# AwesomePeiweiPan/Droid-SLAM_Reserch

Hardware: AMD Instinct MI355X
Metric: BA update iters/sec (2000-edge equivalents; 256 keyframes, 48x64) (higher is better)
Workload: dtype f32; 1 GPU; 256-keyframe / 2000-edge global BA, 48x64, t0=1, lm=1e-5 ep=1e-2 (BASELINE configs[2]); edges_total=2000, solve=fp64 dense Cholesky on device, chol_failed=False

## Files before the change

### droid-slam_reserch_amd/csrc/ba_internal.hpp

```cpp
#pragma once
#include <hip/hip_runtime.h>
#include <stddef.h>
#include <stdint.h>

namespace droid {

constexpr int LIN_THREADS = 256;
constexpr int LIN_PPT = 2;
constexpr int LIN_CP = LIN_THREADS * LIN_PPT;
constexpr int LIN_WAVES = LIN_THREADS / 64;
constexpr int CHOL_NB = 64;
__host__ __device__ inline int chol_ld(int n) { return (n + 1 + 15) & ~15; }
__host__ __device__ inline size_t chol_flag_words(int n) { return 2 * ((size_t)(n + 1 + CHOL_NB - 1) / CHOL_NB) + 8; }
__host__ __device__ inline int chol_tile_index(int nrb, int bi, int bj) { return bj * nrb - bj * (bj - 1) / 2 + (bi - bj); }
__host__ __device__ inline size_t chol_tiles(int n) {
  const int nb = (n + CHOL_NB - 1) / CHOL_NB, nrb = (n + 1 + CHOL_NB - 1) / CHOL_NB;
  return (size_t)chol_tile_index(nrb, nb, nb);
}
__host__ __device__ inline size_t chol_mbuf_offset(int n) { return ((size_t)(n + CHOL_NB - 1) / CHOL_NB) * CHOL_NB * CHOL_NB; }
__host__ __device__ inline size_t chol_lfin_offset(int n) { return 2 * chol_mbuf_offset(n); }
__host__ __device__ inline size_t chol_ldiag_doubles(int n) { return chol_lfin_offset(n) + chol_tiles(n) * CHOL_NB * CHOL_NB; }

__host__ __device__ inline size_t pk_colbase(int n, int J) {
  return (size_t)CHOL_NB * ((size_t)J * (size_t)(n + 1) - (size_t)CHOL_NB * (size_t)J * (size_t)(J - 1) / 2);
}
__host__ __device__ inline int pk_width(int n, int J) { return (n - CHOL_NB * J) < CHOL_NB ? (n - CHOL_NB * J) : CHOL_NB; }
__host__ __device__ inline size_t pk_total(int n) {
  if (n <= 0) return 0;
  const int nb = (n + CHOL_NB - 1) / CHOL_NB;
  return pk_colbase(n, nb - 1) + (size_t)(n + 1 - CHOL_NB * (nb - 1)) * (size_t)pk_width(n, nb - 1);
}
__host__ __device__ inline size_t pk_index(int n, int gi, int gj) {
  const int J = gj / CHOL_NB;
  return pk_colbase(n, J) + (size_t)(gi - CHOL_NB * J) * (size_t)pk_width(n, J) + (size_t)(gj - CHOL_NB * J);
}
__host__ __device__ inline unsigned pk_index32(int n, int gi, int gj) {
  const int J = gj >> 6, c0 = J << 6;
  const int w = (n - c0) < CHOL_NB ? (n - c0) : CHOL_NB;
  return (unsigned)(CHOL_NB * (J * (n + 1) - (CHOL_NB / 2) * J * (J - 1)) + (gi - c0) * w + (gj - c0));
}

enum { HDR_STATUS = 0, HDR_M = 1, HDR_CHOL_FAIL = 2, HDR_NENT = 3, HDR_NWORK = 4,
       HDR_NC1 = 5, HDR_NC2 = 6,
       HDR_WORDS = 16 };
enum { STATUS_BAD_INDEX = 1, STATUS_ETA_ROWS = 2, STATUS_CHOL_FAIL = 4, STATUS_CHOL_STALL = 8 };

struct BaView {
  int E, nbuf, H, W, HW;
  int t0, t1, P, M;
  int n, ld;
  int nch;
  int own0, own1;
  int motion_only;
  int* hdr;
  int* slot_of;
  int* kx;
  int* seg_ptr;
  int* seg_edge;
  int* cursor;
  int* ent_ptr;
  int* ent_row;
  int* ent_pose;
  int* wk_ptr;
  int* order;
  int* xtmp;
  int* cls_list;
  int* gt_ptr;
  double* Gpart;
  int s2_split;
  float* Hpart;
  float* Q;
  float* w;
  float* Erows;
  float* Ebuf;
  float* sy_part[2];
  int sy_ns[2];
  int wide;
  int zsplit;
  float* zpart;
  double* sys;
  double* psys;
  int packed;
  double* xsol;
  float* dx;
  int* bs_flags;
  double* ldiag;
  int* hint;
  int hint_tag;
  int* ov_ready;
};

constexpr int SY_WGS = 1024;
constexpr int S2_WGS = 1536;
constexpr int SF_WGS = 1536;
constexpr int LIN_WGS = 1536;
constexpr int LIN_ZERO_WGS = 192;
constexpr int SF_TP = 64;
constexpr int SW_MID = 256;
constexpr int SW_BIG = 512;
constexpr int tri_tiles16(int rows) { return (rows / 16) * (rows / 16 + 1) / 2; }
constexpr int SY_T1 = tri_tiles16(SW_MID), SY_T2 = tri_tiles16(SW_BIG);
constexpr int SY_FOLD_GROUPS = SY_T1 / 4;

inline size_t ba_carve(BaView& v, void* ws, int E, int nbuf, int H, int W, int t0, int t1, int M) {
  v.E = E; v.nbuf = nbuf; v.H = H; v.W = W; v.HW = H * W;
  v.t0 = t0; v.t1 = t1; v.P = t1 - t0; v.M = M;
  v.n = 6 * v.P; v.ld = chol_ld(v.n);
  v.nch = (v.HW + LIN_CP - 1) / LIN_CP;
  v.own0 = 0; v.own1 = nbuf; v.motion_only = 0;
  v.hint = nullptr; v.hint_tag = 0;
  size_t off = 0;
  char* base = static_cast<char*>(ws);
  auto take = [&](size_t bytes) {
    void* p = base ? base + off : nullptr;
    off += (bytes + 255) & ~size_t(255);
    return p;
  };
  v.hdr = static_cast<int*>(take(sizeof(int) * HDR_WORDS));
  v.slot_of = static_cast<int*>(take(sizeof(int) * (nbuf + 1)));
  v.kx = static_cast<int*>(take(sizeof(int) * (nbuf + 1)));
  v.seg_ptr = static_cast<int*>(take(sizeof(int) * (nbuf + 2)));
  v.seg_edge = static_cast<int*>(take(sizeof(int) * (E + 1)));
  v.cursor = static_cast<int*>(take(sizeof(int) * (nbuf + 2)));
  v.ent_ptr = static_cast<int*>(take(sizeof(int) * (nbuf + 2)));
  v.ent_row = static_cast<int*>(take(sizeof(int) * ((size_t)M + E + 1)));
  v.ent_pose = static_cast<int*>(take(sizeof(int) * ((size_t)M + E + 1)));
  v.wk_ptr = static_cast<int*>(take(sizeof(int) * (nbuf + 2)));
  v.order = static_cast<int*>(take(sizeof(int) * (nbuf + 2)));
  v.gt_ptr = static_cast<int*>(take(sizeof(int) * (nbuf + 2)));
  v.cls_list = static_cast<int*>(take(sizeof(int) * 2 * (nbuf + 2)));
  v.xtmp = static_cast<int*>(take(sizeof(int) * 3 * ((size_t)E + 1)));
  v.Hpart = static_cast<float*>(take(sizeof(float) * ((size_t)E * v.nch * LIN_WAVES * 32 + 32)));
  v.Q = static_cast<float*>(take(sizeof(float) * ((size_t)M * v.HW + 4)));
  v.w = static_cast<float*>(take(sizeof(float) * ((size_t)M * v.HW + 4)));
  v.Erows = nullptr;
  v.wide = (M > 0 && (long)E >= 12l * M && (v.HW % 32) == 0) ? 1 : 0;
  v.Ebuf = nullptr;
  if (v.wide) v.Ebuf = static_cast<float*>(take(sizeof(float) * (6 * ((size_t)M + E) * v.HW + 64)));
  v.sy_part[0] = v.sy_part[1] = nullptr;
  v.sy_ns[0] = v.sy_ns[1] = 0;
  if (v.wide) {
    const int stages = v.HW / 32;
    int nsw = (SY_WGS + M - 1) / M, nsb = (256 + 4 * M - 1) / (4 * M);
    nsw = nsw < 2 ? 2 : (nsw > stages ? stages : nsw);
    nsb = nsb < 2 ? 2 : (nsb > stages ? stages : nsb);
    if (nsw > 16) nsw = 16;
    if (nsb > 16) nsb = 16;
    v.sy_ns[0] = nsw; v.sy_ns[1] = nsb;
    v.sy_part[0] = static_cast<float*>(take(sizeof(float) * ((size_t)M * nsw * SY_T1 * 256 + 64)));
    v.sy_part[1] = static_cast<float*>(take(sizeof(float) * ((size_t)M * nsb * SY_T2 * 256 + 64)));
  }
  v.zsplit = 1;
  if (M > 0) {
    const int z = LIN_WGS / (M * v.nch);
    v.zsplit = z < 1 ? 1 : (z > 8 ? 8 : z);
  }
  v.zpart = nullptr;
  if (v.zsplit > 1) v.zpart = static_cast<float*>(take(sizeof(float) * ((size_t)v.zsplit * M * 8 * v.HW + 64)));
  v.s2_split = 1;
  v.Gpart = nullptr;
  if (M > 0) {
    const int ptiles = (v.HW + 63) / 64;
    int ns = S2_WGS / M;
    v.s2_split = ns < 1 ? 1 : (ns > ptiles ? ptiles : ns);
    size_t tiles = (size_t)E * 7 / 4 + (size_t)M + 1;
    if (tiles > (size_t)28 * M) tiles = (size_t)28 * M;
    v.Gpart = static_cast<double*>(take(sizeof(double) * (tiles * v.s2_split * 256 + 64)));
  }
  v.sys = static_cast<double*>(take(sizeof(double) * ((size_t)(v.n + 1) * v.ld + 8)));
  v.psys = static_cast<double*>(take(sizeof(double) * (pk_total(v.n) + 8)));
  v.packed = 0;
  v.xsol = static_cast<double*>(take(sizeof(double) * ((size_t)v.ld + 1)));
  v.bs_flags = static_cast<int*>(take(sizeof(int) * chol_flag_words(v.n)));
  v.ldiag = static_cast<double*>(take(sizeof(double) * chol_ldiag_doubles(v.n)));
  v.dx = static_cast<float*>(take(sizeof(float) * ((size_t)v.n + 8)));
  v.ov_ready = static_cast<int*>(take(sizeof(int) * ((size_t)(v.n + 1 + CHOL_NB - 1) / CHOL_NB + 8)));
  return off;
}

__host__ __device__ inline int solver_preset_words(const BaView& v) {
  return (int)((reinterpret_cast<const char*>(v.bs_flags) - reinterpret_cast<const char*>(v.xsol)) / 4 +
               (long)chol_flag_words(v.n));
}
__host__ __device__ inline int solver_preset_tiles(const BaView& v) { return v.n > 0 ? (int)chol_tiles(v.n) : 0; }

struct BaLaunchPlan {
  int zero_wgs;
  int asm_units;
  dim3 schur2;
  int sf_split;
  dim3 syrk[2], fold;
};
inline BaLaunchPlan ba_launch_plan(const BaView& v) {
  BaLaunchPlan p;
  p.zero_wgs = LIN_ZERO_WGS;
  p.asm_units = v.E > 0 ? v.E + (solver_preset_words(v) + 1023) / 1024 + solver_preset_tiles(v) : 0;
  p.schur2 = dim3(v.M + (p.asm_units + 4 * v.s2_split - 1) / (4 * v.s2_split), v.s2_split);
  const int tiles = (v.HW + SF_TP - 1) / SF_TP, ns = SF_WGS / (v.M > 0 ? v.M : 1);
  p.sf_split = ns < 1 ? 1 : (ns > tiles ? tiles : ns);
  p.syrk[0] = dim3(v.M, v.sy_ns[0], 1);
  p.syrk[1] = dim3(v.M, v.sy_ns[1], 4);
  p.fold = dim3(v.M, SY_FOLD_GROUPS, 2);
  return p;
}

struct CholSystem {
  double* S; int n, ld; double* x; int* flags; double* ldiag; int* fail;
  explicit CholSystem(const BaView& v)
      : S(v.sys), n(v.n), ld(v.ld), x(v.xsol), flags(v.bs_flags), ldiag(v.ldiag), fail(v.hdr + HDR_CHOL_FAIL) {}
  CholSystem(double* scratch, int n, double* x, int* fail);
  static size_t scratch_doubles(int n);
};

void launch_wave_reduce32_test(const float* in, float* out, hipStream_t s);
void launch_prep(const BaView& v, const int64_t* ii, const int64_t* jj, hipStream_t s);
void launch_unpack_system(const BaView& v, hipStream_t s);
void launch_build_stage(const BaView& v, const BaLaunchPlan& plan, const float* poses, const float* disps,
                        const float* intr, const float* sens, const float* targets, const float* weights,
                        const float* eta, const int64_t* ii, const int64_t* jj, bool motion_only,
                        int stage, hipStream_t s);
void launch_update(const BaView& v, float* poses, float* disps, const float* intr, const float* weights,
                   const int64_t* ii, const int64_t* jj, const double* x, float* dx_out, float* dz_out,
                   bool motion_only, hipStream_t s, int* status_mirror = nullptr);
void launch_chol_preset(const CholSystem& c, hipStream_t s);
bool launch_chol_factor(const CholSystem& c, double lm, double ep, hipStream_t s);
void launch_chol_backsolve(const CholSystem& c, bool factor_single, hipStream_t s);
void launch_chol_solve(const CholSystem& c, double lm, double ep, hipStream_t s, bool preset_done);

void launch_unpack_cols(const BaView& v, int J0, int J1, double lm, double ep, int epoch, hipStream_t s);
bool launch_chol_factor_overlap(const CholSystem& c, const int* ready, int epoch, hipStream_t s);
bool chol_overlap_available(int n);

}
```

### droid-slam_reserch_amd/csrc/ba_kernels.hip

```cpp
#include <hip/hip_runtime.h>
#include <stdint.h>
#include <stdlib.h>

#include "ba_internal.hpp"
#include "se3.hpp"

namespace droid {


__device__ void block_exscan(int* data, int L, int* lds, int* total) {
  const int T = blockDim.x, t = threadIdx.x, lane = t & 63, wave = t >> 6, nw = T >> 6;
  const int per = (L + T - 1) / T;
  const int b = t * per;
  int s = 0;
  for (int k = 0; k < per; k++)
    if (b + k < L) s += data[b + k];
  int incl = s;
#pragma unroll
  for (int off = 1; off < 64; off <<= 1) {
    const int v = __shfl_up(incl, off);
    if (lane >= off) incl += v;
  }
  if (lane == 63) lds[wave] = incl;
  __syncthreads();
  if (wave == 0) {
    int w = (lane < nw) ? lds[lane] : 0;
    int wi = w;
#pragma unroll
    for (int off = 1; off < 64; off <<= 1) {
      const int v = __shfl_up(wi, off);
      if (lane >= off) wi += v;
    }
    if (lane < nw) lds[lane] = wi - w;
    if (lane == nw - 1) *total = wi;
  }
  __syncthreads();
  int run = lds[wave] + incl - s;
  for (int k = 0; k < per; k++)
    if (b + k < L) {
      int v = data[b + k];
      data[b + k] = run;
      run += v;
    }
  __syncthreads();
}

template <int CTRL, int BANKS>
__device__ __forceinline__ float dpp_move(float old, float src) {
  return __int_as_float(__builtin_amdgcn_update_dpp(__float_as_int(old), __float_as_int(src), CTRL, 0xf, BANKS, false));
}
__device__ __forceinline__ float wave_reduce32(float (&v)[32]) {
  constexpr int ROW_SHL4 = 0x104, ROW_SHR4 = 0x114, ROW_ROR8 = 0x128, QUAD_XOR2 = 0x4E, QUAD_XOR1 = 0xB1;
  const int lane = threadIdx.x & 63;
#pragma unroll
  for (int i = 0; i < 16; i++) {
    const auto r = __builtin_amdgcn_permlane32_swap(__float_as_uint(v[2 * i]), __float_as_uint(v[2 * i + 1]), false, false);
    v[i] = __uint_as_float(r[0]) + __uint_as_float(r[1]);
  }
#pragma unroll
  for (int i = 0; i < 8; i++) {
    const auto r = __builtin_amdgcn_permlane16_swap(__float_as_uint(v[2 * i]), __float_as_uint(v[2 * i + 1]), false, false);
    v[i] = __uint_as_float(r[0]) + __uint_as_float(r[1]);
  }
#pragma unroll
  for (int i = 0; i < 4; i++) {
    const float a = dpp_move<ROW_ROR8, 0x3>(v[2 * i + 1], v[2 * i]);
    const float b = dpp_move<ROW_ROR8, 0xC>(v[2 * i], v[2 * i + 1]);
    v[i] = a + b;
  }
#pragma unroll
  for (int i = 0; i < 2; i++) {
    const float a = dpp_move<ROW_SHL4, 0x5>(v[2 * i + 1], v[2 * i]);
    const float b = dpp_move<ROW_SHR4, 0xA>(v[2 * i], v[2 * i + 1]);
    v[i] = a + b;
  }
  {
    const bool hi = lane & 2;
    float keep = hi ? v[1] : v[0];
    float send = hi ? v[0] : v[1];
    v[0] = keep + dpp_move<QUAD_XOR2, 0xF>(send, send);
  }
  return v[0] + dpp_move<QUAD_XOR1, 0xF>(v[0], v[0]);
}

__device__ __forceinline__ int reduce32_index(int lane) {
  return ((lane >> 5) & 1) | (((lane >> 4) & 1) << 1) | (((lane >> 3) & 1) << 2) |
         (((lane >> 2) & 1) << 3) | (((lane >> 1) & 1) << 4);
}

__global__ __launch_bounds__(64) void wave_reduce32_test_kernel(const float* __restrict__ in, float* __restrict__ out) {
  float v[32];
#pragma unroll
  for (int k = 0; k < 32; k++) v[k] = in[threadIdx.x * 32 + k];
  out[threadIdx.x] = wave_reduce32(v);
}
void launch_wave_reduce32_test(const float* in, float* out, hipStream_t s) {
  hipLaunchKernelGGL(wave_reduce32_test_kernel, dim3(1), dim3(64), 0, s, in, out);
}

__device__ __forceinline__ double* sys_at(const BaView& v, int gi, int gj) {
  if (v.packed) {
    unsigned idx = pk_index32(v.n, gi, gj);
    asm volatile("" : "+v"(idx));
    return v.psys + idx;
  }
  return v.sys + (size_t)gi * v.ld + gj;
}

constexpr int SLOT_MAXE = 128;
template <typename S>
struct SlotMetaT {
  int e[SLOT_MAXE];
  int pj[SLOT_MAXE];
  int ent[SLOT_MAXE];
  int flag[SLOT_MAXE];
  S T[SLOT_MAXE][12];
};
typedef SlotMetaT<float> SlotMeta;

constexpr int SF_RB = 96;
constexpr int SY_MAXSPLIT = 16;

constexpr int S2_MAXE = 16;
__device__ __forceinline__ int schur_class(int rows, int nedges, int wide) {
  if (nedges <= S2_MAXE) return 0;
  if (!wide || nedges > SLOT_MAXE || rows > SW_BIG) return 3;
  return rows <= SW_MID ? 1 : 2;
}
__device__ __forceinline__ size_t ebuf_index(int e0, int rows, int HW, int row, int k) {
  return (size_t)6 * e0 * HW + ((size_t)(k >> 5) * rows + row) * 32 + (k & 31);
}
__device__ __forceinline__ int s2_tiles(int nedges) {
  const int ntr = (6 * nedges + 15) / 16;
  return ntr * (ntr + 1) / 2 + 1;
}

template <typename S>
__device__ __forceinline__ void load_slot_meta(SlotMetaT<S>& sm, const BaView& v, const float* __restrict__ poses,
                                               const int64_t* __restrict__ jj, int f, int x0, int cnt,
                                               int ent_base) {
  const int t = threadIdx.x;
  if (t < cnt) {
    const int e = v.seg_edge[x0 + t];
    const int jx = (int)jj[e];
    const RelMat<S> T = rel_pose_mat<S, true>(poses, f, jx);
    sm.e[t] = e;
    sm.pj[t] = jx - v.t0;
    sm.flag[t] = (jx == f) ? 1 : 0;
#pragma unroll
    for (int n = 0; n < 9; n++) sm.T[t][n] = T.R[n];
#pragma unroll
    for (int n = 0; n < 3; n++) sm.T[t][9 + n] = T.t[n];
  }
  __syncthreads();
  if (t < cnt) {
    int a = ent_base;
    for (int u = 0; u < t; u++) a += (sm.pj[u] >= 0 && sm.pj[u] < v.P) ? 1 : 0;
    sm.ent[t] = (sm.pj[t] >= 0 && sm.pj[t] < v.P) ? a : -1;
  }
  __syncthreads();
}

__host__ __device__ inline size_t prep_lds_ints(int nbuf, int E) { return 9 * ((size_t)nbuf + 2) + 4 * ((size_t)E + 1); }

template <bool INLDS>
__global__ __launch_bounds__(1024) void ba_prep_kernel(BaView vg, const int64_t* __restrict__ ii,
                                                        const int64_t* __restrict__ jj) {
  __shared__ int lds[1024];
  __shared__ int tot;
  extern __shared__ int dyn[];
  const int t = threadIdx.x, T = blockDim.x;
  BaView v = vg;
  if (INLDS) {
    int* q = dyn;
    const int nb2 = vg.nbuf + 2, e1 = vg.E + 1;
    v.slot_of = q; q += nb2;
    v.kx = q; q += nb2;
    v.seg_ptr = q; q += nb2;
    v.cursor = q; q += nb2;
    v.ent_ptr = q; q += nb2;
    v.wk_ptr = q; q += nb2;
    v.order = q; q += nb2;
    v.gt_ptr = q; q += nb2;
    q += nb2;
    v.seg_edge = q; q += e1;
    v.xtmp = q;
  }
  const int E = v.E, nbuf = v.nbuf;
  const int w0 = max(v.t0, v.own0), w1 = min(v.t1, v.own1);

  if (t == 0) {
    v.hdr[HDR_STATUS] = 0;
    v.hdr[HDR_CHOL_FAIL] = 0;
  }
  for (int f = t; f < nbuf; f += T) v.slot_of[f] = 0;
  __syncthreads();
  for (int e = t; e < E; e += T) {
    const int64_t i = ii[e], j = jj[e];
    if (i < 0 || i >= nbuf || j < 0 || j >= nbuf)
      atomicOr(&v.hdr[HDR_STATUS], STATUS_BAD_INDEX);
    else
      v.slot_of[i] = 1;
  }
  if (v.motion_only) {
    if (t == 0) {
      v.hdr[HDR_M] = 0;
      v.hdr[HDR_NENT] = 0;
      v.hdr[HDR_NWORK] = 0;
    }
    return;
  }
  for (int f = w0 + t; f < w1; f += T)
    if (f >= 0 && f < nbuf) v.slot_of[f] = 1;
  __syncthreads();
  for (int f = t; f < nbuf; f += T) v.cursor[f] = v.slot_of[f];
  __syncthreads();
  block_exscan(v.cursor, nbuf, lds, &tot);
  const int M = tot;
  for (int f = t; f < nbuf; f += T) {
    if (v.slot_of[f]) {
      v.slot_of[f] = v.cursor[f];
      v.kx[v.cursor[f]] = f;
    } else {
      v.slot_of[f] = -1;
    }
  }
  __syncthreads();
  if (t == 0) {
    v.hdr[HDR_M] = M;
    if (M != v.M) atomicOr(&v.hdr[HDR_STATUS], STATUS_ETA_ROWS);
  }
  const int Ms = min(M, v.M);
  for (int m = t; m <= nbuf; m += T) v.seg_ptr[m] = 0;
  __syncthreads();
  for (int e = t; e < E; e += T) {
    const int64_t i = ii[e], j = jj[e];
    if (i >= 0 && i < nbuf && j >= 0 && j < nbuf) atomicAdd(&v.seg_ptr[v.slot_of[i]], 1);
  }
  __syncthreads();
  block_exscan(v.seg_ptr, nbuf + 1, lds, &tot);
  for (int m = t; m < nbuf; m += T) v.cursor[m] = 0;
  __syncthreads();
  int* utmp = v.xtmp;
  int* xflag = v.xtmp + (E + 1);
  int* xslot = v.xtmp + 2 * (E + 1);
  for (int e = t; e < E; e += T) {
    const int64_t i = ii[e], j = jj[e];
    if (i >= 0 && i < nbuf && j >= 0 && j < nbuf) {
      const int m = v.slot_of[i];
      const int pos = atomicAdd(&v.cursor[m], 1);
      utmp[v.seg_ptr[m] + pos] = e;
    }
  }
  __syncthreads();
  for (int e = t; e < E; e += T) {
    const int64_t i = ii[e], j = jj[e];
    if (i >= 0 && i < nbuf && j >= 0 && j < nbuf) {
      const int m = v.slot_of[i];
      const int a = v.seg_ptr[m], b = v.seg_ptr[m + 1];
      int rank = 0;
      for (int x = a; x < b; x++) rank += (utmp[x] < e) ? 1 : 0;
      const int p = (int)j - v.t0;
      v.seg_edge[a + rank] = e;
      xflag[a + rank] = (p >= 0 && p < v.P) ? 1 : 0;
      xslot[a + rank] = m;
    }
  }
  __syncthreads();
  for (int m = t; m <= nbuf; m += T) v.ent_ptr[m] = 0;
  __syncthreads();
  for (int m = t; m < Ms; m += T) {
    const int f = v.kx[m];
    int c = (f >= w0 && f < w1) ? 1 : 0;
    for (int x = v.seg_ptr[m]; x < v.seg_ptr[m + 1]; x++) c += xflag[x];
    v.ent_ptr[m] = c;
  }
  __syncthreads();
  block_exscan(v.ent_ptr, nbuf + 1, lds, &tot);
  if (t == 0) v.hdr[HDR_NENT] = tot;
  for (int m = t; m < Ms; m += T) {
    const int f = v.kx[m];
    if (f >= w0 && f < w1) {
      v.ent_row[v.ent_ptr[m]] = m;
      v.ent_pose[v.ent_ptr[m]] = f - v.t0;
    }
  }
  for (int x = t; x < v.seg_ptr[Ms]; x += T) {
    if (!xflag[x]) continue;
    const int m = xslot[x];
    const int f = v.kx[m];
    int o = v.ent_ptr[m] + ((f >= w0 && f < w1) ? 1 : 0);
    for (int y = v.seg_ptr[m]; y < x; y++) o += xflag[y];
    const int e = v.seg_edge[x];
    v.ent_row[o] = v.M + e;
    v.ent_pose[o] = (int)jj[e] - v.t0;
  }
  __syncthreads();
  for (int m = t; m <= nbuf; m += T) v.gt_ptr[m] = 0;
  __syncthreads();
  for (int m = t; m < Ms; m += T) {
    const int ne = v.seg_ptr[m + 1] - v.seg_ptr[m];
    v.gt_ptr[m] = (ne > 0 && ne <= S2_MAXE) ? s2_tiles(ne) : 0;
  }
  __syncthreads();
  block_exscan(v.gt_ptr, nbuf + 1, lds, &tot);
  for (int m = t; m < Ms; m += T) v.wk_ptr[m] = v.seg_ptr[m + 1] - v.seg_ptr[m];
  __syncthreads();
  for (int m = t; m < Ms; m += T) {
    const int c = v.wk_ptr[m];
    int rank = 0;
    for (int u = 0; u < Ms; u++) {
      const int cu = v.wk_ptr[u];
      rank += (cu > c || (cu == c && u < m)) ? 1 : 0;
    }
    v.order[rank] = m;
  }
  if (t == 0) v.hdr[HDR_NWORK] = 0;
  if (t < 2) v.hdr[HDR_NC1 + t] = 0;
  __syncthreads();
  int my3 = 0;
  for (int m = t; m < Ms; m += T) {
    const int nent = v.ent_ptr[m + 1] - v.ent_ptr[m];
    const int c = nent > 0 ? schur_class(6 * nent + 1, v.seg_ptr[m + 1] - v.seg_ptr[m], v.wide) : 0;
    v.wk_ptr[m] = c;
    my3 += (c == 3) ? 1 : 0;
  }
  const int n3 = __syncthreads_count(my3);
  if (t == 0 && vg.hint) {
    __hip_atomic_store(vg.hint + 1, n3, __ATOMIC_RELAXED, __HIP_MEMORY_SCOPE_SYSTEM);
    __hip_atomic_store(vg.hint, vg.hint_tag, __ATOMIC_RELEASE, __HIP_MEMORY_SCOPE_SYSTEM);
  }
  for (int m = t; m < Ms; m += T) {
    const int c = v.wk_ptr[m];
    if (c != 1 && c != 2) continue;
    int pos = 0, after = 0;
    for (int u = 0; u < Ms; u++) {
      const int same = v.wk_ptr[u] == c;
      pos += (same && u < m) ? 1 : 0;
      after += (same && u > m) ? 1 : 0;
    }
    vg.cls_list[(c - 1) * (nbuf + 2) + pos] = m;
    if (after == 0) v.hdr[HDR_NC1 + c - 1] = pos + 1;
  }
  if (INLDS) {
    __syncthreads();
    for (int f = t; f <= nbuf; f += T) {
      vg.slot_of[f] = (f < nbuf) ? v.slot_of[f] : -1;
      vg.kx[f] = v.kx[f];
      vg.seg_ptr[f] = v.seg_ptr[f];
      vg.ent_ptr[f] = v.ent_ptr[f];
      vg.gt_ptr[f] = v.gt_ptr[f];
      vg.order[f] = v.order[f];
    }
    for (int x = t; x < E; x += T) vg.seg_edge[x] = v.seg_edge[x];
  }
}

template <bool DEPTH, bool EROWS, bool ZSPLIT, bool FULL>
__global__ __launch_bounds__(LIN_THREADS, 3) void ba_lin_kernel(
    BaView v, const float* __restrict__ poses, const float* __restrict__ disps,
    const float* __restrict__ intrinsics, const float* __restrict__ disps_sens,
    const float* __restrict__ targets, const float* __restrict__ weights,
    const float* __restrict__ eta, const int64_t* __restrict__ ii, const int64_t* __restrict__ jj, int zero_base) {
  __shared__ SlotMetaT<double> sm;
  const int tid = threadIdx.x, lane = tid & 63, wave = tid >> 6;
  const int HW = v.HW, W = v.W;
  const int chunk = blockIdx.y;
  if ((int)blockIdx.x >= zero_base) {
    if (blockIdx.y != 0 || blockIdx.z != 0) return;
    const int nz = (int)gridDim.x - zero_base;
    if (v.packed) {
      double2* p = reinterpret_cast<double2*>(v.psys);
      const size_t n2 = pk_total(v.n) / 2;
      for (size_t c = (size_t)((int)blockIdx.x - zero_base) * LIN_THREADS + tid; c < n2; c += (size_t)nz * LIN_THREADS)
        p[c] = make_double2(0.0, 0.0);
      return;
    }
    for (int row = (int)blockIdx.x - zero_base; row <= v.n; row += nz) {
      double2* p = reinterpret_cast<double2*>(v.sys + (size_t)row * v.ld);
      const int n2 = (row == v.n) ? v.ld / 2 : (row + 2) / 2;
      for (int c = tid; c < n2; c += LIN_THREADS) p[c] = make_double2(0.0, 0.0);
    }
    return;
  }
  int xb, xe, f = -1, m = -1;
  if (DEPTH) {
    if ((int)blockIdx.x >= min(v.hdr[HDR_M], v.M)) return;
    m = v.order[blockIdx.x];
    f = v.kx[m];
    xb = v.seg_ptr[m];
    xe = v.seg_ptr[m + 1];
  } else {
    xb = blockIdx.x;
    xe = xb + 1;
    const int64_t i0 = ii[xb], j0 = jj[xb];
    if (i0 < 0 || i0 >= v.nbuf || j0 < 0 || j0 >= v.nbuf) return;
  }
  const Intr K = {intrinsics[0], intrinsics[1], intrinsics[2], intrinsics[3]};
  int xs = xb, xend = xe;
  if (DEPTH && ZSPLIT) {
    const int per = (xe - xb + (int)gridDim.z - 1) / (int)gridDim.z;
    xs = min(xe, xb + (int)blockIdx.z * per);
    xend = min(xe, xs + per);
  }

  bool emit = false, has_self = false;
  int e0 = 0, erows = 0;
  if (DEPTH && EROWS) {
    e0 = v.ent_ptr[m];
    const int nent = v.ent_ptr[m + 1] - e0;
    erows = 6 * nent;
    const int cls = schur_class(6 * nent + 1, xe - xb, 1);
    emit = (cls == 1 || cls == 2);
    has_self = nent > 0 && (v.ent_row[e0] < v.M);
  }
  float selfacc[LIN_PPT][6];
#pragma unroll
  for (int p = 0; p < LIN_PPT; p++)
#pragma unroll
    for (int n = 0; n < 6; n++) selfacc[p][n] = 0.f;

  int pix[LIN_PPT];
  float disp[LIN_PPT], Cacc[LIN_PPT], wacc[LIN_PPT];
  double X0d[LIN_PPT], X1d[LIN_PPT];
#pragma unroll
  for (int p = 0; p < LIN_PPT; p++) {
    pix[p] = chunk * LIN_CP + p * LIN_THREADS + tid;
    Cacc[p] = 0.f;
    wacc[p] = 0.f;
    disp[p] = 0.f;
    if (DEPTH && (FULL || pix[p] < HW)) disp[p] = disps[(size_t)f * HW + pix[p]];
    const int kk = (FULL || pix[p] < HW) ? pix[p] : 0;
    X0d[p] = ((double)(kk % W) - (double)K.cx) / (double)K.fx;
    X1d[p] = ((double)(kk / W) - (double)K.cy) / (double)K.fy;
  }

  float in_cur[LIN_PPT][4], in_nxt[LIN_PPT][4];
  bool have_next = false;
  auto fetch_edge = [&](int e, float (&dst)[LIN_PPT][4]) {
    const float* tg = targets + (size_t)e * 2 * HW;
    const float* wg = weights + (size_t)e * 2 * HW;
#pragma unroll
    for (int p = 0; p < LIN_PPT; p++) {
      const bool ok = FULL || pix[p] < HW;
      const int k = ok ? pix[p] : 0;
      dst[p][0] = ok ? tg[k] : 0.f;
      dst[p][1] = ok ? tg[HW + k] : 0.f;
      dst[p][2] = ok ? wg[k] : 0.f;
      dst[p][3] = ok ? wg[HW + k] : 0.f;
    }
  };
  for (int x = xs; x < xend; x++) {
    if (DEPTH && (x == xs || ((x - xb) % SLOT_MAXE) == 0)) {
      if (x > xs) __syncthreads();
      const int cb = xb + ((x - xb) / SLOT_MAXE) * SLOT_MAXE;
      load_slot_meta(sm, v, poses, jj, f, cb, min(SLOT_MAXE, xe - cb), (EROWS && has_self) ? 1 : 0);
    }
    const int xl = DEPTH ? (x - xb) % SLOT_MAXE : 0;
    const int e = DEPTH ? sm.e[xl] : x;
    const int ix = DEPTH ? f : (int)ii[e];
    double Rt[12];
    bool stereo;
    if (DEPTH) {
#pragma unroll
      for (int n = 0; n < 12; n++) Rt[n] = sm.T[xl][n];
      stereo = sm.flag[xl] != 0;
    } else {
      const int jx = (int)jj[e];
      const RelMat<double> T = rel_pose_mat<double, true>(poses, ix, jx);
#pragma unroll
      for (int n = 0; n < 9; n++) Rt[n] = T.R[n];
#pragma unroll
      for (int n = 0; n < 3; n++) Rt[9 + n] = T.t[n];
      stereo = (ix == jx);
    }
    if (!have_next) fetch_edge(e, in_cur);
    else {
#pragma unroll
      for (int p = 0; p < LIN_PPT; p++)
#pragma unroll
        for (int c = 0; c < 4; c++) in_cur[p][c] = in_nxt[p][c];
    }
    have_next = false;
    if (DEPTH && x + 1 < xend && xl + 1 < SLOT_MAXE) {
      fetch_edge(sm.e[xl + 1], in_nxt);
      have_next = true;
    }
    float acc[32];
#pragma unroll
    for (int k = 0; k < 32; k++) acc[k] = 0.f;
#pragma unroll
    for (int p = 0; p < LIN_PPT; p++) {
      if (FULL ? (chunk * LIN_CP + p * LIN_THREADS < HW) : (pix[p] < HW)) {
        const int k = pix[p];
        const float d = DEPTH ? disp[p] : disps[(size_t)ix * HW + k];
        const PixLin L = linearize_pixel_d(K, Rt, Rt + 9, X0d[p], X1d[p], d, in_cur[p][0], in_cur[p][1]);
        float wu = L.valid * (0.001f * in_cur[p][2]);
        float wv = L.valid * (0.001f * in_cur[p][3]);
        if (DEPTH) {
          Cacc[p] += wu * L.Jzu * L.Jzu + wv * L.Jzv * L.Jzv;
          wacc[p] += wu * L.ru * L.Jzu + wv * L.rv * L.Jzv;
        }
        if (stereo) {
          wu = 0.f;
          wv = 0.f;
        }
        int l = 0;
#pragma unroll
        for (int a = 0; a < 6; a++) {
          const float wa_u = wu * L.Ju[a], wa_v = wv * L.Jv[a];
#pragma unroll
          for (int b = 0; b <= a; b++) {
            acc[l] += wa_u * L.Ju[b] + wa_v * L.Jv[b];
            l++;
          }
          acc[21 + a] += wa_u * L.ru + wa_v * L.rv;
        }
        if (DEPTH && EROWS && emit) {
          const float su = wu * L.Jzu, sv = wv * L.Jzv;
          float eij[6];
#pragma unroll
          for (int n = 0; n < 6; n++) eij[n] = su * L.Ju[n] + sv * L.Jv[n];
          const int a = sm.ent[xl];
          if (a >= 0) {
#pragma unroll
            for (int n = 0; n < 6; n++) v.Ebuf[ebuf_index(e0, erows, HW, 6 * a + n, k)] = eij[n];
          }
          if (has_self) {
            float eii[6];
            adjT_mat(Rt, Rt + 9, eij, eii);
#pragma unroll
            for (int n = 0; n < 6; n++) selfacc[p][n] -= eii[n];
          }
        }
      }
    }
    const float tot = wave_reduce32(acc);
    if ((lane & 1) == 0) v.Hpart[(((size_t)e * v.nch + chunk) * LIN_WAVES + wave) * 32 + reduce32_index(lane)] = tot;
  }

  if (DEPTH && ZSPLIT) {
#pragma unroll
    for (int p = 0; p < LIN_PPT; p++) {
      if (FULL || pix[p] < HW) {
        float* zp = v.zpart + (((size_t)blockIdx.z * v.M + m) * 8) * HW + pix[p];
        zp[0] = Cacc[p];
        zp[(size_t)HW] = wacc[p];
#pragma unroll
        for (int n = 0; n < 6; n++) zp[(size_t)(2 + n) * HW] = selfacc[p][n];
      }
    }
    return;
  }
  if (DEPTH) {
    const float alpha = 0.05f;
#pragma unroll
    for (int p = 0; p < LIN_PPT; p++) {
      if (FULL || pix[p] < HW) {
        const int k = pix[p];
        const size_t o = (size_t)m * HW + k;
        const float sens = disps_sens[(size_t)f * HW + k];
        const float ms = sens > 0.f ? 1.f : 0.f;
        const float C = Cacc[p] + ms * alpha + (1.f - ms) * eta[o];
        const float w = wacc[p] - ms * alpha * (disp[p] - sens);
        v.Q[o] = 1.0f / C;
        v.w[o] = w;
        if (EROWS && emit && has_self) {
#pragma unroll
          for (int n = 0; n < 6; n++) v.Ebuf[ebuf_index(e0, erows, HW, n, k)] = selfacc[p][n];
        }
      }
    }
  }
}

__global__ __launch_bounds__(256) void ba_lin_finish_kernel(BaView v, const float* __restrict__ disps,
                                                            const float* __restrict__ disps_sens,
                                                            const float* __restrict__ eta) {
  if ((int)blockIdx.x >= min(v.hdr[HDR_M], v.M)) return;
  const int m = blockIdx.x, HW = v.HW;
  const int k = blockIdx.y * 256 + threadIdx.x;
  if (k >= HW) return;
  const int f = v.kx[m];
  float s[8] = {0.f, 0.f, 0.f, 0.f, 0.f, 0.f, 0.f, 0.f};
  for (int z = 0; z < v.zsplit; z++) {
    const float* zp = v.zpart + (((size_t)z * v.M + m) * 8) * HW + k;
#pragma unroll
    for (int q = 0; q < 8; q++) s[q] += zp[(size_t)q * HW];
  }
  const float alpha = 0.05f;
  const size_t o = (size_t)m * HW + k;
  const float sens = disps_sens[(size_t)f * HW + k], disp = disps[(size_t)f * HW + k];
  const float ms = sens > 0.f ? 1.f : 0.f;
  v.Q[o] = 1.0f / (s[0] + ms * alpha + (1.f - ms) * eta[o]);
  v.w[o] = s[1] - ms * alpha * (disp - sens);
  if (v.wide) {
    const int e0 = v.ent_ptr[m], nent = v.ent_ptr[m + 1] - e0;
    const int cls = schur_class(6 * nent + 1, v.seg_ptr[m + 1] - v.seg_ptr[m], 1);
    if ((cls == 1 || cls == 2) && nent > 0 && v.ent_row[e0] < v.M) {
#pragma unroll
      for (int n = 0; n < 6; n++) v.Ebuf[ebuf_index(e0, 6 * nent, HW, n, k)] = s[2 + n];
    }
  }
}

struct AssembleScratch {
  double hj[6][6], vj[6], A[6][6], hij[6][6];
};
__device__ __forceinline__ void assemble_unit(const BaView& v, const float* __restrict__ poses, const int64_t* __restrict__ ii,
// ... 844 lines not shown
    c2 = __builtin_amdgcn_mfma_f32_16x16x32_bf16(a2[1], b2[0], c2, 0, 0, 0);
    c = __builtin_amdgcn_mfma_f32_16x16x32_bf16(a[0], b[0], c, 0, 0, 0);
    c2 = __builtin_amdgcn_mfma_f32_16x16x32_bf16(a2[0], b2[0], c2, 0, 0, 0);
    t += c;
    t2 += c2;
  };
  auto mm1 = [&](const bf16x8 (&a)[3], const bf16x8 (&b)[3], f32x4& t) {
    f32x4 c = __builtin_amdgcn_mfma_f32_16x16x32_bf16(a[0], b[2], zero4, 0, 0, 0);
    c = __builtin_amdgcn_mfma_f32_16x16x32_bf16(a[2], b[0], c, 0, 0, 0);
    c = __builtin_amdgcn_mfma_f32_16x16x32_bf16(a[1], b[1], c, 0, 0, 0);
    c = __builtin_amdgcn_mfma_f32_16x16x32_bf16(a[0], b[1], c, 0, 0, 0);
    c = __builtin_amdgcn_mfma_f32_16x16x32_bf16(a[1], b[0], c, 0, 0, 0);
    c = __builtin_amdgcn_mfma_f32_16x16x32_bf16(a[0], b[0], c, 0, 0, 0);
    t += c;
  };
  auto multiply = [&](int buf) {
    const u32x4* P = PL + buf * 12 * NR;
    auto frag = [&](int chunk) { return __builtin_bit_cast(bf16x8, P[chunk]); };
#pragma unroll
    for (int u = 0; u < MAXS; u++) {
      if (mysup[u] >= 0) {
        bf16x8 a0[3], a1[3], b0[3], b1[3];
#pragma unroll
        for (int p = 0; p < 3; p++) {
          a0[p] = frag(offl + offa[u] + 4 * p * NR);
          b0[p] = frag(offl + offb[u] + 4 * p * NR);
        }
        if (second[u]) {
#pragma unroll
          for (int p = 0; p < 3; p++) a1[p] = frag(offl + offa[u] + 16 + 4 * p * NR);
          mm2(a0, b0, acc[u][0], a1, b0, acc[u][2]);
#pragma unroll
          for (int p = 0; p < 3; p++) b1[p] = frag(offl + offb[u] + 16 + 4 * p * NR);
          if (upper[u]) mm2(a0, b1, acc[u][1], a1, b1, acc[u][3]);
          else mm1(a1, b1, acc[u][3]);
        } else if (upper[u]) {
#pragma unroll
          for (int p = 0; p < 3; p++) b1[p] = frag(offl + offb[u] + 16 + 4 * p * NR);
          mm2(a0, b0, acc[u][0], a0, b1, acc[u][1]);
        } else {
          mm1(a0, b0, acc[u][0]);
        }
      }
    }
  };

  auto lds_barrier = [&]() { __syncthreads(); };
  if constexpr (!DBUF) {
    load_q(st_beg);
    load_stage(st_beg, 0);
    for (int st = st_beg; st < st_end; st++) {
      lds_barrier();
      store_stage(0, 0);
      lds_barrier();
      load_q(st + 1);
      load_stage(st + 1, 0);
      multiply(0);
    }
  } else {
    load_q(st_beg);
    load_stage(st_beg, 0);
    load_stage(st_beg + 1, 1);
    store_stage(0, 0);
    load_q(st_beg + 1);
    load_stage(st_beg + 2, 0);
    lds_barrier();
    const bool mul_first = (wave & 1) != 0;
    for (int st = st_beg; st < st_end; st += 2) {
      if (mul_first) multiply(0);
      store_stage(1, 1);
      load_q(st + 2);
      load_stage(st + 3, 1);
      if (!mul_first) multiply(0);
      lds_barrier();
      if (mul_first && st + 1 < st_end) multiply(1);
      store_stage(0, 0);
      load_q(st + 3);
      load_stage(st + 4, 0);
      if (!mul_first && st + 1 < st_end) multiply(1);
      lds_barrier();
    }
  }
  float* part = v.sy_part[CLS - 1] + ((size_t)(wlin % count) * nrange + range) * (size_t)((CLS == 1 ? SY_T1 : SY_T2) * 256);
#pragma unroll
  for (int u = 0; u < MAXS; u++) {
    if (mysup[u] >= 0) {
      int sa, sb;
      tri_coords(mysup[u], sa, sb);
#pragma unroll
      for (int q = 0; q < 4; q++) {
        const int ta = 2 * sa + (q >> 1), tb = 2 * sb + (q & 1);
        if (ta >= ntr || tb > ta) continue;
        *reinterpret_cast<f32x4*>(part + (size_t)(ta * (ta + 1) / 2 + tb) * 256 + 4 * lane) = acc[u][q];
      }
    }
  }
}

__global__ __launch_bounds__(256) void ba_syrk_fold_kernel(BaView v, int wgs1, int wgs2) {
  const int cls = (int)blockIdx.z + 1;
  const int count = min(v.hdr[HDR_NC1 + cls - 1], v.M);
  const int pos = (int)blockIdx.x;
  if (pos >= count) return;
  const int tmax = cls == 1 ? SY_T1 : SY_T2;
  const int stages_total = v.HW / SY_TPX;
  const int nrange = max(1, min(min((cls == 1 ? wgs1 : wgs2) / count, SY_MAXSPLIT), stages_total));
  const int spw = (stages_total + nrange - 1) / nrange;
  const int nused = (stages_total + spw - 1) / spw;
  const int m = v.cls_list[(cls - 1) * (v.nbuf + 2) + pos];
  const int tid = threadIdx.x, lane = tid & 63, wave = tid >> 6;
  const int e0 = v.ent_ptr[m], nent = v.ent_ptr[m + 1] - e0;
  const int R = 6 * nent;
  const int ntr = (R + 1 + 15) / 16, ntiles = ntr * (ntr + 1) / 2;
  __shared__ int s_pose[SLOT_MAXE + 2];
  for (int i = tid; i < nent; i += (int)blockDim.x) s_pose[i] = v.ent_pose[e0 + i];
  __syncthreads();
  const float* part = v.sy_part[cls - 1] + (size_t)pos * nrange * tmax * 256;
  const int r = lane & 15, g = lane >> 4;
  for (int ti = (int)blockIdx.y * 4 + wave; ti < ntiles; ti += 4 * (int)gridDim.y) {
    int ta, tb;
    tri_coords(ti, ta, tb);
    double sum[4] = {0.0, 0.0, 0.0, 0.0};
    for (int rg = 0; rg < nused; rg++) {
      const f32x4 pv = *reinterpret_cast<const f32x4*>(part + ((size_t)rg * tmax + ti) * 256 + 4 * lane);
#pragma unroll
      for (int x = 0; x < 4; x++) sum[x] += (double)pv[x];
    }
    const int lj = 16 * tb + r;
    if (lj >= R) continue;
    const int gj = 6 * s_pose[lj / 6] + lj % 6;
#pragma unroll
    for (int x = 0; x < 4; x++) {
      const int li = 16 * ta + 4 * g + x;
      if (li > R) continue;
      const double val = -sum[x];
      if (li == R) {
        atomicAdd(sys_at(v, v.n, gj), val);
        continue;
      }
      const int gi = 6 * s_pose[li / 6] + li % 6;
      if (ta == tb) {
        if (gi >= gj) atomicAdd(sys_at(v, gi, gj), val);
      } else {
        if (gi > gj) atomicAdd(sys_at(v, gi, gj), val);
        else if (gi < gj) atomicAdd(sys_at(v, gj, gi), val);
        else atomicAdd(sys_at(v, gi, gj), 2.0 * val);
      }
    }
  }
}

constexpr int BSUB_PPT = 1;

__global__ __launch_bounds__(256) void ba_backsub_kernel(
    BaView v, const float* __restrict__ poses, float* __restrict__ disps,
    const float* __restrict__ intrinsics, const float* __restrict__ weights,
    const int64_t* __restrict__ ii, const int64_t* __restrict__ jj, const double* __restrict__ xsol,
    float* __restrict__ dz_out) {
  __shared__ SlotMetaT<double> sm;
  __shared__ float dxs[SLOT_MAXE][6];
  if ((int)blockIdx.x >= min(v.hdr[HDR_M], v.M)) return;
  const int m = v.order[blockIdx.x];
  const int HW = v.HW;
  const int f = v.kx[m];
  const Intr K = {intrinsics[0], intrinsics[1], intrinsics[2], intrinsics[3]};
  int kpix[BSUB_PPT];
  float disp[BSUB_PPT];
  double acc[BSUB_PPT];
  double bx0[BSUB_PPT], bx1[BSUB_PPT];
#pragma unroll
  for (int p = 0; p < BSUB_PPT; p++) {
    kpix[p] = (blockIdx.y * BSUB_PPT + p) * 256 + threadIdx.x;
    disp[p] = kpix[p] < HW ? disps[(size_t)f * HW + kpix[p]] : 0.f;
    acc[p] = 0.0;
    const int kk = kpix[p] < HW ? kpix[p] : 0;
    bx0[p] = ((double)(kk % v.W) - (double)K.cx) / (double)K.fx;
    bx1[p] = ((double)(kk / v.W) - (double)K.cy) / (double)K.fy;
  }
  const int pf = f - v.t0;
  const int e0 = v.ent_ptr[m];
  const bool has_self = (v.ent_ptr[m + 1] > e0) && (v.ent_row[e0] < v.M);
  const bool self_on = has_self && pf > 0;
  const bool failed = v.hdr[HDR_CHOL_FAIL] != 0;
  float dxi[6] = {0.f, 0.f, 0.f, 0.f, 0.f, 0.f};
  if (self_on && !failed)
    for (int n = 0; n < 6; n++) dxi[n] = (float)xsol[6 * pf + n];
  const int x_beg = v.seg_ptr[m], nedges = v.seg_ptr[m + 1] - x_beg;
  for (int c0 = 0; c0 < nedges; c0 += SLOT_MAXE) {
    const int cnt = min(SLOT_MAXE, nedges - c0);
    if (c0 > 0) __syncthreads();
    load_slot_meta(sm, v, poses, jj, f, x_beg + c0, cnt, 0);
    if (threadIdx.x < cnt) {
      const int pj = sm.pj[threadIdx.x];
      const bool on = pj > 0 && pj < v.P;
      float c[6];
      for (int n = 0; n < 6; n++) c[n] = (on && !failed) ? (float)xsol[6 * pj + n] : 0.f;
      if (self_on) {
        const double* T = sm.T[threadIdx.x];
        for (int k = 0; k < 6; k++) {
          float ek[6] = {0.f, 0.f, 0.f, 0.f, 0.f, 0.f}, col[6];
          ek[k] = 1.f;
          adjT_mat(T, T + 9, ek, col);
          float z = 0.f;
          for (int n = 0; n < 6; n++) z += col[n] * dxi[n];
          c[k] -= z;
        }
      }
      for (int n = 0; n < 6; n++) dxs[threadIdx.x][n] = c[n];
      sm.ent[threadIdx.x] = on ? 1 : 0;
    }
    __syncthreads();
    float wnext[BSUB_PPT][2];
    auto fetch_w = [&](int x) {
      const float* wg = weights + (size_t)sm.e[min(x, cnt - 1)] * 2 * HW;
#pragma unroll
      for (int p = 0; p < BSUB_PPT; p++) {
        const int kk = kpix[p] < HW ? kpix[p] : 0;
        wnext[p][0] = wg[kk];
        wnext[p][1] = wg[HW + kk];
      }
    };
    fetch_w(0);
    for (int x = 0; x < cnt; x++) {
      float wraw[BSUB_PPT][2];
#pragma unroll
      for (int p = 0; p < BSUB_PPT; p++) {
        const bool ok = kpix[p] < HW;
        wraw[p][0] = ok ? wnext[p][0] : 0.f;
        wraw[p][1] = ok ? wnext[p][1] : 0.f;
      }
      fetch_w(x + 1);
      const bool edge_on = sm.ent[x] != 0;
      if (!(edge_on || self_on)) continue;
      double T[12];
#pragma unroll
      for (int n = 0; n < 12; n++) T[n] = sm.T[x][n];
#pragma unroll
      for (int p = 0; p < BSUB_PPT; p++) {
        float eij[6];
        e_row(K, T, sm.flag[x] != 0, bx0[p], bx1[p], disp[p], wraw[p][0], wraw[p][1], eij);
        double dw = 0.0;
#pragma unroll
        for (int n = 0; n < 6; n++) dw += (double)eij[n] * (double)dxs[x][n];
        acc[p] += dw;
      }
    }
  }
#pragma unroll
  for (int p = 0; p < BSUB_PPT; p++) {
    if (kpix[p] >= HW) continue;
    const size_t o = (size_t)m * HW + kpix[p];
    const float dz = (float)((double)v.Q[o] * ((double)v.w[o] - acc[p]));
    if (dz_out) dz_out[o] = dz;
    disps[(size_t)f * HW + kpix[p]] = disp[p] + dz;
  }
}

__global__ void ba_pose_retr_kernel(BaView v, float* __restrict__ poses, const double* __restrict__ xsol,
                                    float* __restrict__ dx_out, int* __restrict__ status_mirror) {
  const int p = blockIdx.x * blockDim.x + threadIdx.x;
  const int fl = v.hdr[HDR_CHOL_FAIL];
  const bool failed = fl != 0;
  if (p == 0) {
    int st = v.hdr[HDR_STATUS];
    if (failed) {
      st |= (fl >= 2) ? STATUS_CHOL_STALL : STATUS_CHOL_FAIL;
      atomicOr(&v.hdr[HDR_STATUS], (fl >= 2) ? STATUS_CHOL_STALL : STATUS_CHOL_FAIL);
    }
    if (status_mirror) {
      __hip_atomic_store(status_mirror + 1, v.hdr[HDR_M], __ATOMIC_RELAXED, __HIP_MEMORY_SCOPE_SYSTEM);
      __hip_atomic_store(status_mirror, st, __ATOMIC_RELAXED, __HIP_MEMORY_SCOPE_SYSTEM);
      if (st & (STATUS_BAD_INDEX | STATUS_ETA_ROWS | STATUS_CHOL_STALL)) {
        const int cnt = __hip_atomic_load(status_mirror + 2, __ATOMIC_RELAXED, __HIP_MEMORY_SCOPE_SYSTEM);
        const int bits = __hip_atomic_load(status_mirror + 3, __ATOMIC_RELAXED, __HIP_MEMORY_SCOPE_SYSTEM);
        __hip_atomic_store(status_mirror + 3, bits | st, __ATOMIC_RELAXED, __HIP_MEMORY_SCOPE_SYSTEM);
        __hip_atomic_store(status_mirror + 2, cnt + 1, __ATOMIC_RELEASE, __HIP_MEMORY_SCOPE_SYSTEM);
      }
    }
  }
  if (p >= v.P) return;
  const int k = v.t0 + p;
  float xi[6], t[3], q[4], tn[3], qn[4];
  for (int n = 0; n < 6; n++) {
    xi[n] = failed ? 0.f : (float)xsol[6 * p + n];
    v.dx[6 * p + n] = xi[n];
    if (dx_out) dx_out[6 * p + n] = xi[n];
  }
  for (int n = 0; n < 3; n++) t[n] = poses[7 * k + n];
  for (int n = 0; n < 4; n++) q[n] = poses[7 * k + 3 + n];
  retr_se3(xi, t, q, tn, qn);
  for (int n = 0; n < 3; n++) poses[7 * k + n] = tn[n];
  for (int n = 0; n < 4; n++) poses[7 * k + 3 + n] = qn[n];
}

template <bool DAMP>
__global__ __launch_bounds__(256) void ba_unpack_kernel(BaView v, int J0, double lm, double ep) {
  const int J = J0 + (int)blockIdx.y, w = pk_width(v.n, J), c0 = CHOL_NB * J;
  const int c = 2 * ((int)threadIdx.x & 31);
  for (int row = c0 + 8 * (int)blockIdx.x + ((int)threadIdx.x >> 5); row <= v.n; row += 8 * (int)gridDim.x) {
    if (c < w) {
      double2 x = *reinterpret_cast<const double2*>(v.psys + pk_colbase(v.n, J) + (size_t)(row - c0) * w + c);
      if (DAMP && row < v.n) {
        if (c0 + c == row) x.x += ep + lm * x.x;
        else if (c0 + c + 1 == row) x.y += ep + lm * x.y;
      }
      *reinterpret_cast<double2*>(v.sys + (size_t)row * v.ld + c0 + c) = x;
    }
  }
}
__global__ void ba_set_ready_kernel(int* __restrict__ ready, int b0, int b1, int epoch) {
  const int b = b0 + (int)threadIdx.x;
  if (b < b1) __hip_atomic_store(ready + b, epoch, __ATOMIC_RELEASE, __HIP_MEMORY_SCOPE_AGENT);
}

void launch_unpack_system(const BaView& v, hipStream_t s) {
  if (v.n <= 0) return;
  const int nb = (v.n + CHOL_NB - 1) / CHOL_NB;
  hipLaunchKernelGGL(ba_unpack_kernel<false>, dim3(min((v.n + 8) / 8, 64), nb), dim3(256), 0, s, v, 0, 0.0, 0.0);
}

void launch_unpack_cols(const BaView& v, int J0, int J1, double lm, double ep, int epoch, hipStream_t s) {
  if (J1 <= J0) return;
  hipLaunchKernelGGL(ba_unpack_kernel<true>, dim3(min((v.n + 8 - CHOL_NB * J0) / 8, 64), J1 - J0), dim3(256), 0, s, v, J0, lm, ep);
  hipLaunchKernelGGL(ba_set_ready_kernel, dim3(1), dim3(64), 0, s, v.ov_ready, J0, J1, epoch);
}

void launch_prep(const BaView& v, const int64_t* ii, const int64_t* jj, hipStream_t s) {
  const size_t lds_bytes = sizeof(int) * prep_lds_ints(v.nbuf, v.E);
  static bool attr_set = false;
  if (lds_bytes <= 150 * 1024) {
    if (!attr_set) {
      (void)hipFuncSetAttribute((const void*)ba_prep_kernel<true>, hipFuncAttributeMaxDynamicSharedMemorySize, 150 * 1024);
      attr_set = true;
    }
    hipLaunchKernelGGL(ba_prep_kernel<true>, dim3(1), dim3(1024), lds_bytes, s, v, ii, jj);
  } else {
    hipLaunchKernelGGL(ba_prep_kernel<false>, dim3(1), dim3(1024), 0, s, v, ii, jj);
  }
}

template <bool FULL>
static auto lin_kernel_of(bool wide, bool zsplit) {
  return wide ? (zsplit ? ba_lin_kernel<true, true, true, FULL> : ba_lin_kernel<true, true, false, FULL>)
              : (zsplit ? ba_lin_kernel<true, false, true, FULL> : ba_lin_kernel<true, false, false, FULL>);
}
static auto lin_kernel_of(bool wide, bool zsplit, bool full) {
  return full ? lin_kernel_of<true>(wide, zsplit) : lin_kernel_of<false>(wide, zsplit);
}

void launch_build_stage(const BaView& v, const BaLaunchPlan& plan, const float* poses, const float* disps,
                        const float* intr, const float* sens, const float* targets, const float* weights,
                        const float* eta, const int64_t* ii, const int64_t* jj, bool motion_only,
                        int stage, hipStream_t s) {
  const bool depth = !motion_only && v.M > 0;
  const bool full = v.HW % LIN_CP == 0;
  switch (stage) {
    case 0:
      if (depth) {
        const dim3 g(v.M + plan.zero_wgs, v.nch, v.zsplit), b(LIN_THREADS);
        const auto lin = lin_kernel_of(v.wide != 0, v.zsplit > 1, full);
        hipLaunchKernelGGL(lin, g, b, 0, s, v, poses, disps, intr, sens, targets, weights, eta, ii, jj, v.M);
        if (v.zsplit > 1)
          hipLaunchKernelGGL(ba_lin_finish_kernel, dim3(v.M, (v.HW + 255) / 256), dim3(256), 0, s, v, disps, sens, eta);
      } else if (v.E > 0) {
        const auto lin = full ? ba_lin_kernel<false, false, false, true> : ba_lin_kernel<false, false, false, false>;
        hipLaunchKernelGGL(lin, dim3(v.E + plan.zero_wgs, v.nch), dim3(LIN_THREADS), 0, s, v, poses,
                           disps, intr, sens, targets, weights, eta, ii, jj, v.E);
      } else {
        if (v.packed) (void)hipMemsetAsync(v.psys, 0, sizeof(double) * pk_total(v.n), s);
        else (void)hipMemsetAsync(v.sys, 0, sizeof(double) * (size_t)(v.n + 1) * v.ld, s);
      }
      break;
    case 1:
      if (v.E > 0 && !depth)
        hipLaunchKernelGGL(ba_assemble_kernel, dim3(plan.asm_units), dim3(64), 0, s, v, poses, ii, jj);
      break;
    case 2:
      if (depth) {
        const int wide = v.wide;
        hipLaunchKernelGGL(ba_schur2_kernel, plan.schur2, dim3(256), 0, s, v, poses, disps, intr, weights, ii, jj,
                           wide, plan.asm_units);
        hipLaunchKernelGGL(ba_schur_fold_kernel, dim3(v.M), dim3(1024), 0, s, v, poses, jj, v.s2_split);
        bool none3 = false;
        if (v.hint) {
          const int tag = __atomic_load_n(v.hint, __ATOMIC_ACQUIRE);
          none3 = tag == v.hint_tag && __atomic_load_n(v.hint + 1, __ATOMIC_RELAXED) == 0;
        }
        if (!none3)
          hipLaunchKernelGGL(ba_schur_fused_kernel, dim3(v.M, plan.sf_split), dim3(256), 0, s, v, poses, disps,
                             intr, weights, ii, jj, wide);
        if (wide) {
          hipLaunchKernelGGL((ba_syrk3_kernel<SW_MID, 12, 1, 1, true, true>), plan.syrk[0], dim3(768), 0, s, v);
          hipLaunchKernelGGL((ba_syrk3_kernel<SW_BIG, 8, 2, 4, false, false>), plan.syrk[1], dim3(512), 0, s, v);
          hipLaunchKernelGGL(ba_syrk_fold_kernel, plan.fold, dim3(256), 0, s, v, v.M * v.sy_ns[0], v.M * v.sy_ns[1]);
        }
      }
      break;
  }
// ... 13 lines not shown
```

Baseline: 1993 iters/s.

## Cache per-edge pose rows in global table and prefetch them in backsub

The linearization kernel now writes each edge's relative pose, edge id, pose index and flag into a 128-byte-aligned global EdgeRow table. The backsub loop reads these rows through a wave-uniform pointer and software-pipelines the next edge's transform and weight address alongside the current edge's work, instead of reading from LDS each iteration. Launch bounds are also given an occupancy hint. This adds a global table write in linearize and more register pressure from double-buffered transforms, and it relies on the table being filled before backsub runs. Backsub still calls load_slot_meta, so that redundant work remains.

Measured after the change: 2006 iters/s, median of 6. Within noise of the previous version (+0.7%).

```diff
diff --git a/droid-slam_reserch_amd/csrc/ba_internal.hpp b/droid-slam_reserch_amd/csrc/ba_internal.hpp
--- a/droid-slam_reserch_amd/csrc/ba_internal.hpp
+++ b/droid-slam_reserch_amd/csrc/ba_internal.hpp
@@ -44,6 +44,12 @@
        HDR_NC1 = 5, HDR_NC2 = 6,
        HDR_WORDS = 16 };
 enum { STATUS_BAD_INDEX = 1, STATUS_ETA_ROWS = 2, STATUS_CHOL_FAIL = 4, STATUS_CHOL_STALL = 8 };
+
+struct alignas(128) EdgeRow {
+  double T[12];
+  int e, pj, ent, flag;
+};
+static_assert(sizeof(EdgeRow) == 128, "one 128-byte row per edge");
 
 struct BaView {
   int E, nbuf, H, W, HW;
@@ -88,6 +94,7 @@
   int* hint;
   int hint_tag;
   int* ov_ready;
+  EdgeRow* etab;
 };
 
 constexpr int SY_WGS = 1024;
@@ -175,6 +182,8 @@
   v.ldiag = static_cast<double*>(take(sizeof(double) * chol_ldiag_doubles(v.n)));
   v.dx = static_cast<float*>(take(sizeof(float) * ((size_t)v.n + 8)));
   v.ov_ready = static_cast<int*>(take(sizeof(int) * ((size_t)(v.n + 1 + CHOL_NB - 1) / CHOL_NB + 8)));
+  v.etab = nullptr;
+  if (M > 0) v.etab = static_cast<EdgeRow*>(take(sizeof(EdgeRow) * (size_t)E));
   return off;
 }
 
diff --git a/droid-slam_reserch_amd/csrc/ba_kernels.hip b/droid-slam_reserch_amd/csrc/ba_kernels.hip
--- a/droid-slam_reserch_amd/csrc/ba_kernels.hip
+++ b/droid-slam_reserch_amd/csrc/ba_kernels.hip
@@ -159,6 +159,20 @@
     sm.ent[t] = (sm.pj[t] >= 0 && sm.pj[t] < v.P) ? a : -1;
   }
   __syncthreads();
+}
+
+__device__ __forceinline__ void store_edge_rows(const SlotMetaT<double>& sm, const BaView& v, int x0, int cnt, int xs,
+                                                int xend) {
+  const int t = threadIdx.x;
+  if (t < cnt && x0 + t >= xs && x0 + t < xend) {
+    EdgeRow* row = v.etab + (x0 + t);
+#pragma unroll
+    for (int n = 0; n < 12; n++) row->T[n] = sm.T[t][n];
+    row->e = sm.e[t];
+    row->pj = sm.pj[t];
+    row->ent = sm.ent[t];
+    row->flag = sm.flag[t];
+  }
 }
 
 __host__ __device__ inline size_t prep_lds_ints(int nbuf, int E) { return 9 * ((size_t)nbuf + 2) + 4 * ((size_t)E + 1); }
@@ -455,6 +469,7 @@
       if (x > xs) __syncthreads();
       const int cb = xb + ((x - xb) / SLOT_MAXE) * SLOT_MAXE;
       load_slot_meta(sm, v, poses, jj, f, cb, min(SLOT_MAXE, xe - cb), (EROWS && has_self) ? 1 : 0);
+      if (chunk == 0) store_edge_rows(sm, v, cb, min(SLOT_MAXE, xe - cb), xs, xend);
     }
     const int xl = DEPTH ? (x - xb) % SLOT_MAXE : 0;
     const int e = DEPTH ? sm.e[xl] : x;
@@ -1605,13 +1620,14 @@
 
 constexpr int BSUB_PPT = 1;
 
-__global__ __launch_bounds__(256) void ba_backsub_kernel(
+__global__ __launch_bounds__(256, 5) void ba_backsub_kernel(
     BaView v, const float* __restrict__ poses, float* __restrict__ disps,
     const float* __restrict__ intrinsics, const float* __restrict__ weights,
     const int64_t* __restrict__ ii, const int64_t* __restrict__ jj, const double* __restrict__ xsol,
     float* __restrict__ dz_out) {
   __shared__ SlotMetaT<double> sm;
   __shared__ float dxs[SLOT_MAXE][6];
+  const EdgeRow* __restrict__ etab = v.etab;
   if ((int)blockIdx.x >= min(v.hdr[HDR_M], v.M)) return;
   const int m = v.order[blockIdx.x];
   const int HW = v.HW;
@@ -1641,6 +1657,7 @@
   const int x_beg = v.seg_ptr[m], nedges = v.seg_ptr[m + 1] - x_beg;
   for (int c0 = 0; c0 < nedges; c0 += SLOT_MAXE) {
     const int cnt = min(SLOT_MAXE, nedges - c0);
+    const EdgeRow* __restrict__ rows = etab + __builtin_amdgcn_readfirstlane(x_beg + c0);
     if (c0 > 0) __syncthreads();
     load_slot_meta(sm, v, poses, jj, f, x_beg + c0, cnt, 0);
     if (threadIdx.x < cnt) {
@@ -1664,8 +1681,8 @@
     }
     __syncthreads();
     float wnext[BSUB_PPT][2];
-    auto fetch_w = [&](int x) {
-      const float* wg = weights + (size_t)sm.e[min(x, cnt - 1)] * 2 * HW;
+    auto fetch_w = [&](int e) {
+      const float* wg = weights + (size_t)e * 2 * HW;
 #pragma unroll
       for (int p = 0; p < BSUB_PPT; p++) {
         const int kk = kpix[p] < HW ? kpix[p] : 0;
@@ -1673,7 +1690,12 @@
         wnext[p][1] = wg[HW + kk];
       }
     };
-    fetch_w(0);
+    fetch_w(rows[0].e);
+    int e_nxt = rows[min(1, cnt - 1)].e;
+    double T[12];
+#pragma unroll
+    for (int n = 0; n < 12; n++) T[n] = rows[0].T[n];
+    int pj = rows[0].pj, flag = rows[0].flag;
     for (int x = 0; x < cnt; x++) {
       float wraw[BSUB_PPT][2];
 #pragma unroll
@@ -1682,21 +1704,29 @@
         wraw[p][0] = ok ? wnext[p][0] : 0.f;
         wraw[p][1] = ok ? wnext[p][1] : 0.f;
       }
-      fetch_w(x + 1);
-      const bool edge_on = sm.ent[x] != 0;
-      if (!(edge_on || self_on)) continue;
-      double T[12];
-#pragma unroll
-      for (int n = 0; n < 12; n++) T[n] = sm.T[x][n];
-#pragma unroll
-      for (int p = 0; p < BSUB_PPT; p++) {
-        float eij[6];
-        e_row(K, T, sm.flag[x] != 0, bx0[p], bx1[p], disp[p], wraw[p][0], wraw[p][1], eij);
-        double dw = 0.0;
-#pragma unroll
-        for (int n = 0; n < 6; n++) dw += (double)eij[n] * (double)dxs[x][n];
-        acc[p] += dw;
-      }
+      fetch_w(e_nxt);
+      const EdgeRow* __restrict__ rn = rows + min(x + 1, cnt - 1);
+      double Tn[12];
+#pragma unroll
+      for (int n = 0; n < 12; n++) Tn[n] = rn->T[n];
+      const int pjn = rn->pj, flagn = rn->flag;
+      e_nxt = rows[min(x + 2, cnt - 1)].e;
+      const bool edge_on = pj > 0 && pj < v.P;
+      if (edge_on || self_on) {
+#pragma unroll
+        for (int p = 0; p < BSUB_PPT; p++) {
+          float eij[6];
+          e_row(K, T, flag != 0, bx0[p], bx1[p], disp[p], wraw[p][0], wraw[p][1], eij);
+          double dw = 0.0;
+#pragma unroll
+          for (int n = 0; n < 6; n++) dw += (double)eij[n] * (double)dxs[x][n];
+          acc[p] += dw;
+        }
+      }
+#pragma unroll
+      for (int n = 0; n < 12; n++) T[n] = Tn[n];
+      pj = pjn;
+      flag = flagn;
     }
   }
 #pragma unroll
```
